# salvatore373/Humanoid-Navigation-using-MPC-LDCBF

Measured on AMD Instinct MI355X. Metric: MPC-step QP solves/sec (batch) at N=8, 10 obstacles, higher is better.
Workload: dtype f64

## Files before the change

### humanoid-navigation-using-mpc-ldcbf_amd/csrc/lipmpc_comm.hpp

```cpp
#pragma once
#include "lipmpc_types.hpp"

namespace lipmpc_dev {

#ifndef STREAM_UNROLL
#define STREAM_UNROLL 5
#endif
template <int I, int E, class F> __device__ __forceinline__ void static_for(F&& f) {
  if constexpr (I < E) {
    f(std::integral_constant<int, I>{});
    static_for<I + 1, E>(f);
  }
}
template <int I, int E, class F> __device__ __forceinline__ void static_rfor(F&& f) {
  if constexpr (I > E) {
    f(std::integral_constant<int, I - 1>{});
    static_rfor<I - 1, E>(f);
  }
}

__device__ __forceinline__ int fresh(int x) {
  asm volatile("" : "+v"(x));
  return x;
}
template <int CTRL, int BANK = 0xf, class T> __device__ __forceinline__ T dpp0(T x) {
  return __builtin_amdgcn_mov_dpp(x, CTRL, 0xf, BANK, true);
}
template <int M, class T> __device__ __forceinline__ T row_xor(T x) {
  if constexpr (M == 1) return dpp0<0xB1>(x);
  else if constexpr (M == 2) return dpp0<0x4E>(x);
  else if constexpr (M == 4) {
    T r = __builtin_amdgcn_mov_dpp(x, 0x104, 0xf, 0x5, false);
    return __builtin_amdgcn_update_dpp(r, x, 0x114, 0xf, 0xA, false);
  } else return dpp0<0x128>(x);
}
template <class T> __device__ __forceinline__ void rowpair(T v, T& even_rep, T& odd_rep) {
  if constexpr (sizeof(T) == 8) {
    const unsigned long long u = __builtin_bit_cast(unsigned long long, v);
    const unsigned lo = (unsigned)u, hi = (unsigned)(u >> 32);
    const auto a = __builtin_amdgcn_permlane16_swap(lo, lo, false, false);
    const auto b = __builtin_amdgcn_permlane16_swap(hi, hi, false, false);
    even_rep = __builtin_bit_cast(T, ((unsigned long long)b[0] << 32) | a[0]);
    odd_rep = __builtin_bit_cast(T, ((unsigned long long)b[1] << 32) | a[1]);
  } else {
    const unsigned u = __builtin_bit_cast(unsigned, v);
    const auto a = __builtin_amdgcn_permlane16_swap(u, u, false, false);
    const unsigned a0 = a[0], a1 = a[1];
    even_rep = __builtin_bit_cast(T, a0);
    odd_rep = __builtin_bit_cast(T, a1);
  }
}
template <class T> __device__ __forceinline__ T rowswap(T v) {
  T e, o;
  rowpair(v, e, o);
  const T r = (fresh(threadIdx.x) & 16) ? e : o;
  return r;
}
template <int G, int M, class T> __device__ __forceinline__ T gxor(T x) {
  if constexpr (M < 16) return row_xor<M>(x);
  else return rowswap(x);
}
template <int G, int J> __device__ __forceinline__ double gbcast(double x) {
  const double t = __builtin_amdgcn_mov_dpp(x, 0x150 + (J & 15), 0xf, 0xf, false);
  if constexpr (G == 16) return t;
  else {
    double e, o;
    rowpair(t, e, o);
    return (J < 16) ? e : o;
  }
}
template <int G, int D> __device__ __forceinline__ double gup(double x, int lane_) {
  const int lane = (G == 16) ? lane_ : fresh(lane_);
  if constexpr (G == 16) return dpp0<0x110 + D>(x);
  else if constexpr (D == 16) { const double w = rowswap(x); return (lane & 16) ? w : 0.0; }
  else {
    const double t = dpp0<0x120 + D>(x);
    const double w = rowswap(t);
    return ((lane & 15) >= D) ? t : ((lane & 16) ? w : 0.0);
  }
}
template <int G, int D> __device__ __forceinline__ double gdown(double x, int lane_) {
  const int lane = (G == 16) ? lane_ : fresh(lane_);
  if constexpr (G == 16) return dpp0<0x100 + D>(x);
  else if constexpr (D == 16) { const double w = rowswap(x); return (lane & 16) ? 0.0 : w; }
  else {
    const double t = dpp0<0x120 + (16 - D)>(x);
    const double w = rowswap(t);
    return ((lane & 15) + D < 16) ? t : ((lane & 16) ? 0.0 : w);
  }
}

template <int G> __device__ __forceinline__ double gsum(double x) {
  x += gxor<G, 1>(x); x += gxor<G, 2>(x); x += gxor<G, 4>(x); x += gxor<G, 8>(x);
  if constexpr (G == 32) x += gxor<G, 16>(x);
  return x;
}
__device__ __forceinline__ double vmax(double a, double b) {
  double r;
  asm("v_max_f64 %0, %1, %2" : "=v"(r) : "v"(a), "v"(b));
  return r;
}
__device__ __forceinline__ double vmin(double a, double b) {
  double r;
  asm("v_min_f64 %0, %1, %2" : "=v"(r) : "v"(a), "v"(b));
  return r;
}
__device__ __forceinline__ double vmax_abs(double m, double x) {
  double r;
  asm("v_max_f64 %0, %1, |%2|" : "=v"(r) : "v"(m), "v"(x));
  return r;
}
__device__ __forceinline__ double vmax0_abs(double x) {
  double r;
  asm("v_max_f64 %0, 0, |%1|" : "=v"(r) : "v"(x));
  return r;
}
__device__ __forceinline__ double vmax0(double x) {
  double r;
  asm("v_max_f64 %0, 0, %1" : "=v"(r) : "v"(x));
  return r;
}
template <int G> __device__ __forceinline__ double gmin(double x) {
  x = vmin(x, gxor<G, 1>(x)); x = vmin(x, gxor<G, 2>(x));
  x = vmin(x, dpp0<0x124>(x));
  x = vmin(x, gxor<G, 8>(x));
  if constexpr (G == 32) x = vmin(x, gxor<G, 16>(x));
  return x;
}
template <int G> __device__ __forceinline__ int gmin_int(int x) {
  x = min(x, gxor<G, 1>(x)); x = min(x, gxor<G, 2>(x)); x = min(x, dpp0<0x124>(x)); x = min(x, gxor<G, 8>(x));
  if constexpr (G == 32) x = min(x, gxor<G, 16>(x));
  return x;
}
template <int G> __device__ __forceinline__ double gmax(double x) {
  x = vmax(x, gxor<G, 1>(x)); x = vmax(x, gxor<G, 2>(x));
  x = vmax(x, dpp0<0x124>(x));
  x = vmax(x, gxor<G, 8>(x));
  if constexpr (G == 32) x = vmax(x, gxor<G, 16>(x));
  return x;
}
template <int G, int M> __device__ __forceinline__ void gargmin_step(double& v, int& i) {
  const double ov = gxor<G, M>(v);
  const int oi = gxor<G, M>(i);
  const bool take = (ov < v) || (ov == v && oi < i);
  v = take ? ov : v;
  i = take ? oi : i;
}
template <int G> __device__ __forceinline__ void gargmin(double& v, int& i) {
  gargmin_step<G, 1>(v, i); gargmin_step<G, 2>(v, i); gargmin_step<G, 4>(v, i); gargmin_step<G, 8>(v, i);
  if constexpr (G == 32) gargmin_step<G, 16>(v, i);
}
template <int G> __device__ __forceinline__ double prefix_excl2(double v, int lane) {
  double s = v;
  s += gup<G, 2>(s, lane); s += gup<G, 4>(s, lane); s += gup<G, 8>(s, lane);
  if constexpr (G == 32) s += gup<G, 16>(s, lane);
  return s - v;
}
template <int G> __device__ __forceinline__ double suffix_excl2(double v, int lane) {
  double s = v;
  s += gdown<G, 2>(s, lane); s += gdown<G, 4>(s, lane); s += gdown<G, 8>(s, lane);
  if constexpr (G == 32) s += gdown<G, 16>(s, lane);
  return s - v;
}
__device__ __forceinline__ double fast_rsqrt(double x) {
  double y = __builtin_amdgcn_rsq(x);
  y = y * fma(-0.5 * x * y, y, 1.5);
  y = y * fma(-0.5 * x * y, y, 1.5);
  return y;
}
__device__ __forceinline__ double fast_rcp(double x) {
  double y = __builtin_amdgcn_rcp(x);
  return fma(fma(-x, y, 1.0), y, y);
}
__device__ __forceinline__ double chain_rcp(double x) { return fast_rcp(x); }

template <int J> __device__ __forceinline__ double fmac_bcast_self(double acc, double mult) {
  asm("s_nop 1\n\tv_fmac_f64_dpp %0, %0, %1 row_newbcast:%2 row_mask:0xf bank_mask:0xf" : "+v"(acc) : "v"(mult), "n"(J));
  return acc;
}
__device__ __forceinline__ void dpp_fence() { asm volatile("s_nop 4"); }
#include "lipmpc_fused_steps.inc"

__device__ __forceinline__ double zero_unless(bool c, double x) {
  const unsigned long long u = __builtin_bit_cast(unsigned long long, x);
  const unsigned hi = c ? (unsigned)(u >> 32) : 0u;
  return __builtin_bit_cast(double, ((unsigned long long)hi << 32) | (unsigned)u);
}
#ifdef LIPMPC_PHASE_TIMING
constexpr int PH_WORDS = 32;
__device__ __forceinline__ void ph_mark(unsigned long long* acc, int k, int G) {
  const unsigned long long now = wall_clock64();
  const unsigned long long live = __ballot(1);
  if ((int)threadIdx.x == __ffsll((long long)live) - 1) {
    const unsigned long long dt = now - acc[31];
    acc[k] += dt;
    if (__popcll(live) <= G) acc[12 + k] += dt;
    acc[31] = now;
  }
  __builtin_amdgcn_fence(__ATOMIC_ACQ_REL, "workgroup");
  __builtin_amdgcn_wave_barrier();
}
#define PH_DECL __shared__ unsigned long long ph_acc_[PH_WORDS];                                                   \
  if (threadIdx.x == 0) { for (int k_ = 0; k_ < PH_WORDS; ++k_) ph_acc_[k_] = 0ull; ph_acc_[31] = in.t_start_wall; }     \
  __builtin_amdgcn_fence(__ATOMIC_ACQ_REL, "workgroup"); __builtin_amdgcn_wave_barrier();
#define PH(k) ph_mark(ph_acc_, k, G);
#else
#define PH_DECL
#define PH(k)
#endif
constexpr int WAVE = 64;
__device__ __forceinline__ void wave_sync() {
  __builtin_amdgcn_fence(__ATOMIC_ACQ_REL, "workgroup");
  __builtin_amdgcn_wave_barrier();
}
__device__ __forceinline__ double lds_read_here(const double* p) {
  return *(const volatile __attribute__((address_space(3))) double*)p;
}
struct RowFlags {
  unsigned m = 0u;
  __device__ __forceinline__ bool operator[](int i) const { return (m >> i) & 1u; }
  __device__ __forceinline__ void set(int i, bool v) { m = v ? (m | (1u << i)) : (m & ~(1u << i)); }
};

}
```

### humanoid-navigation-using-mpc-ldcbf_amd/csrc/lipmpc_solve.hpp

```cpp
#pragma once
#include "lipmpc_front.hpp"

namespace lipmpc_dev {

template <int G, int NOBS_L, int NVAR = G, bool LEAN = false, bool RECORD = false>
__device__ __forceinline__ StepOut step_solve(
    const KArgs& P, const StepIn& in, const FrontOut<G>& F, const double (*obs)[4], const int* perm,
    double* __restrict__ U, double* __restrict__ X, double* __restrict__ obj_out, int32_t* __restrict__ status_out,
    int32_t* __restrict__ iters_out, unsigned long long* __restrict__ active_out,
    unsigned long long* __restrict__ working_out,
    double* __restrict__ diag, WarmIO* __restrict__ warm, int32_t* __restrict__ cost_out) {
  static_assert(NVAR == G || (G == 16 && NVAR == 8), "variable slots: all lanes, or the first 8 of a 16-lane group");
  constexpr int NMAX = NVAR / 2;
  constexpr int LMAX = G / 2;
  constexpr int NV = NVAR;
  constexpr int GPW = 64 / G;
  constexpr bool STREAM = NOBS_L > 7;
  constexpr int NOBS_R = STREAM ? 0 : NOBS_L;
  constexpr int NOBS_S = STREAM ? NOBS_L : 0;
  constexpr int NR = R_CBF + NOBS_R;
  constexpr int MAXOBS = 2 * NOBS_L;
  constexpr int MAXWORDS = 16;
  constexpr bool FUSED = (G == 16);
  constexpr bool FUSED32 = (G == 32);
  constexpr bool FUSED32_SOLVE = FUSED32 && NOBS_L <= 2 && !LEAN;

  __shared__ double lds_P[GPW][LMAX][2][2];
  __shared__ unsigned long long lds_act[GPW][MAXWORDS];
  __shared__ double lds_mu[GPW][2];
  __shared__ double lds_sz[GPW][NOBS_S > 0 ? NOBS_S : 1][G][2];

  PH_DECL
  const int tid = threadIdx.x;
  const int lane = tid & (G - 1);
  const int grp = tid / G;
  const bool valid = in.valid;
  const long pb = in.pb;
  const int N = P.N;
  const int a = lane >> 1;
  const int c = lane & 1;
  const bool var_on = a < N;
  const double sgn_a = (a & 1) ? -1.0 : 1.0;
  const double kap = P.kappa;

  const double p0x = in.p0x, v0x = in.v0x, p0y = in.p0y, v0y = in.v0y, th0 = in.th0;
  const double gx = in.gx, gy = in.gy, foot0 = in.foot0, delta = in.delta;
  const double p0c = c ? p0y : p0x, v0c = c ? v0y : v0x, gc = c ? gy : gx;

  const double th_r = F.th_r, th_v = F.th_v, om_a = F.om_a, theta1 = F.theta1, omega0 = F.omega0;
  const double s_own = F.s_own, c_own = F.c_own;
  (void)th_r; (void)th_v;
  const double s_oth = gxor<G, 1>(s_own), c_oth = gxor<G, 1>(c_own);
  const double sr = c ? s_oth : s_own, cr = c ? c_oth : c_own, sv = c ? s_own : s_oth, cv = c ? c_own : c_oth;
  const double foot_r = (a & 1) ? -foot0 : foot0;
  const double foot_v = -foot_r;
  const double on = var_on ? 1.0 : 0.0;
  const double ro = on * cr, rq = on * (c ? -sr : sr);
  const double wo = on * (c ? cv * foot_v : cv), wq = on * (c ? -sv : sv);
  const double cm = (c == 0) ? on : 0.0;
  const double kap_l = on * kap;

  const int front_flag = F.front_flag;
  const double n_ball = F.n_ball, s_ball = F.s_ball;
  const bool ball = (lane == 1) && (n_ball > 0.0);
  const double ball_w = ball ? n_ball - 1.0 : 0.0;

  double oo[NOBS_R > 0 ? NOBS_R : 1], oq[NOBS_R > 0 ? NOBS_R : 1], ob[NOBS_R > 0 ? NOBS_R : 1];
  RowFlags pres;
#pragma unroll
  for (int t = 0; t < NOBS_R; ++t) {
    const int j = 2 * t + c;
    const bool there = var_on && ((double)(a + 1) >= obs[j][3]);
    const double ex = obs[j][0], ey = obs[j][1];
    oo[t] = there ? (c ? ey : ex) : 0.0; oq[t] = there ? (c ? ex : ey) : 0.0;
    ob[t] = there ? obs[j][2] : -1.0;
    pres.set(R_CBF + t, there);
  }
  unsigned pbits = 0u;
#pragma unroll
  for (int t = 0; t < NOBS_S; ++t)
    if (var_on && (double)(a + 1) >= obs[2 * t + c][3]) pbits |= 1u << t;
  auto s_obs = [&](int t, double& ex, double& ey, double& b) {
    const double* o = obs[2 * t + c];
    ex = o[0]; ey = o[1]; b = o[2];
  };
  auto s_pm = [&](int t) -> double { return ((pbits >> t) & 1u) ? 1.0 : 0.0; };
  pres.set(R_RU, var_on); pres.set(R_RL, var_on); pres.set(R_VU, var_on); pres.set(R_VL, var_on);
  pres.set(R_M, (var_on && (c == 0)) || ball);

  const double hi_r = P.l_max[c], lo_r = P.l_min[c];
  const double hi_v = c ? in.vmax_y : in.vmax_x, lo_v = P.v_min[c];
  const double hi_m = in.vmax_x - in.alpha_over_pi * fabs(om_a);
  const double p0q = c ? p0x : p0y, v0q = c ? v0x : v0y;
  const double r_c = (c ? foot_r * P.ell : 0.0) - ((a == 0) ? (ro * p0c + rq * p0q) : 0.0);
  const double w_c = wo * (-sgn_a * (v0c + kap * p0c)) + wq * (-sgn_a * (v0q + kap * p0q));

  int n_rows_l = __popc(pbits);
#pragma unroll
  for (int i = 0; i < NR; ++i) n_rows_l += pres[i] ? 1 : 0;
  const double m_rows = gsum<G>((double)n_rows_l) + fmax(n_ball - 1.0, 0.0);
  const double inv_m = 1.0 / fmax(m_rows, 1.0);

#include "lipmpc_solve_ops.inc"
#include "lipmpc_solve_ipm.inc"
#include "lipmpc_solve_finish.inc"
#include "lipmpc_solve_outputs.inc"
  StepOut r;
  r.status = status; r.iters = iters; r.theta1 = theta1; r.omega0 = omega0; r.obj = objv;
  r.ux = gbcast<G, 0>(u); r.uy = gbcast<G, 1>(u);
  return r;
}


}
```

### humanoid-navigation-using-mpc-ldcbf_amd/csrc/lipmpc_solve_finish.inc

```
  if (ball) { pres.set(R_M, false); s[R_M] = 1.0; z[R_M] = 0.0; }
  if (warm_on) {
    wave_sync();
    warm->lds[lane] = q;
#pragma unroll
    for (int i = 0; i < NR && i < WARM_ROWS; ++i) {
      if constexpr (RECORD) warm->lds[(1 + i) * G + lane] = pres[i] ? z[i] : 0.0;
      else warm->lds[(1 + i) * G + lane] = z[i];
    }
    wave_sync();
  }
  const CanonicalRows ci_of{a, c, N, P, perm};
  auto ci_s = [&](int t) -> int { return ci_of.ldcbf(t); };

  double marg_l = INFINITY;
  const bool want_diag = diag != nullptr;
  RowFlags act;
  unsigned abits = 0u;
#pragma unroll
  for (int i = 0; i < NR; ++i) {
    if (want_diag && pres[i]) marg_l = fmin(marg_l, fabs(log(z[i] / (FIN_IDENT * s[i]))));
    act.set(i, pres[i] && (z[i] > FIN_IDENT * s[i]));
  }
  if constexpr (STREAM) {
#pragma unroll STREAM_UNROLL
    for (int t = 0; t < NOBS_S; ++t) {
      if ((pbits >> t) & 1u) {
        const double st = lds_sz[grp][t][lane][0], zt = lds_sz[grp][t][lane][1];
        if (want_diag) marg_l = fmin(marg_l, fabs(log(zt / (FIN_IDENT * st))));
        if (zt > FIN_IDENT * st) abits |= 1u << t;
      }
    }
  }
  const unsigned fbits = abits;
  const double margin = gmin<G>(marg_l);
  double diag_rounds = 0.0, diag_eres = 0.0, diag_cert = 0.0;

  const bool ipm_ok = (status == LIPMPC_STATUS_SOLVED) && (m_rows > 0.0);
  if (!(P.flags & LIPMPC_FLAG_INTERIOR)) {
    bool fin_done = !ipm_ok;
    bool certified = false;
    double rho = FIN_RHO;
    double xf = q;
    double qf = q;
    double y[NR];
#pragma unroll
    for (int i = 0; i < NR; ++i) y[i] = act[i] ? z[i] : 0.0;
    if constexpr (STREAM) {
#pragma unroll STREAM_UNROLL
      for (int t = 0; t < NOBS_S; ++t)
        if (!((abits >> t) & 1u)) lds_sz[grp][t][lane][1] = 0.0;
    }
    auto s_slack = [&](int t, double fx, double fy) -> double {
#pragma clang fp contract(off)
      double ex, ey, bb;
      s_obs(t, ex, ey, bb);
      return ex * fx + ey * fy - bb;
    };
    auto s_ratio = [&](int t, double fx, double fy, double ddx, double ddy) -> double {
#pragma clang fp contract(off)
      double ex, ey, bb;
      s_obs(t, ex, ey, bb);
      const double sl = ex * fx + ey * fy - bb, gd = -(ex * ddx + ey * ddy);
      const bool cand = gd > FIN_GD_MIN;
      return cand ? fmax(sl + gd, 0.0) * fast_rcp(gd) : INFINITY;
    };
    for (int rnd = 0; rnd < P.fin_rounds; ++rnd) {
      if (__all(fin_done)) break;
      double d[NR];
#pragma unroll
      for (int i = 0; i < NR; ++i) d[i] = act[i] ? rho : 0.0;
      double cxs = 0.0, cxys = 0.0, cys = 0.0;
      if constexpr (STREAM) {
#pragma unroll STREAM_UNROLL
        for (int t = 0; t < NOBS_S; ++t) {
          if ((abits >> t) & 1u) {
            double ex, ey, bb;
            s_obs(t, ex, ey, bb);
            cxs = fma(rho * ex, ex, cxs); cxys = fma(rho * ex, ey, cxys); cys = fma(rho * ey, ey, cys);
          }
        }
      }
      PH(9)
      K_rows(d, cxs, cxys, cys);
      const bool fok = factor();
      PH(7)
      qf = xf;
      double eres = INFINITY, rd_g = 0.0, r_g = 0.0;
      for (int in = 0; in <= FIN_INNER; ++in) {
        slack_values(qf);
        const double fx = cx_, fy = cy_;
        double wr[NR], rmax_l = 0.0;
#pragma unroll
        for (int i = 0; i < NR; ++i) {
          const double r = act[i] ? -slk[i] : 0.0;
          wr[i] = -d[i] * slk[i];
          rmax_l = i == 0 ? vmax0_abs(r) : vmax_abs(rmax_l, r);
        }
        double ayx = 0.0, ayy = 0.0, awx = 0.0, awy = 0.0;
        if constexpr (STREAM) {
#pragma unroll STREAM_UNROLL
          for (int t = 0; t < NOBS_S; ++t) {
            if ((abits >> t) & 1u) {
              double ex, ey, bb;
              s_obs(t, ex, ey, bb);
              const double r = -(ex * fx + ey * fy - bb);
              const double yt = lds_sz[grp][t][lane][1];
              rmax_l = fmax(rmax_l, fabs(r));
              ayx = fma(ex, yt, ayx); ayy = fma(ey, yt, ayy);
              awx = fma(ex, rho * r, awx); awy = fma(ey, rho * r, awy);
            }
          }
        }
        const double gty = GT_rows(y, ayx, ayy);
        const double rd = var_on ? (2.0 * (qf - gc) + gty) : 0.0;
        const double eprev = eres;
        rd_g = gmax<G>(fabs(rd));
        r_g = gmax<G>(rmax_l);
        eres = vmax(rd_g, r_g);
        const bool stop = (eres <= FIN_INNER_TOL) || (in == FIN_INNER) || (eres <= FIN_EPS && eres > FIN_STALL * eprev);
        if (__all(stop || fin_done)) break;
        const double dq = solve(-rd - GT_rows(wr, awx, awy));
        double dl[NR];
        rows_dir(dq, dl);
        if (!stop && !fin_done) {
          qf += dq;
#pragma unroll
          for (int i = 0; i < NR; ++i) y[i] = fma(d[i], dl[i] - slk[i], y[i]);
          if constexpr (STREAM) {
            const double ddx = cx_, ddy = cy_;
#pragma unroll STREAM_UNROLL
            for (int t = 0; t < NOBS_S; ++t) {
              if ((abits >> t) & 1u) {
                double ex, ey, bb;
                s_obs(t, ex, ey, bb);
                const double slk_t = ex * fx + ey * fy - bb, dl_t = -(ex * ddx + ey * ddy);
                lds_sz[grp][t][lane][1] += rho * (dl_t - slk_t);
              }
            }
          }
        }
      }
      PH(8)
      const double fx = cx_, fy = cy_;
      const double dd = qf - xf;
      double gd[NR], rr[NR];
      rows_dir(dd, gd);
      const double ddx = cx_, ddy = cy_;
      double rbest = INFINITY;
#pragma unroll
      for (int i = 0; i < NR; ++i) {
        const bool cand = pres[i] & !act[i] & (gd[i] > FIN_GD_MIN);
        rr[i] = cand ? fmax(slk[i] + gd[i], 0.0) * fast_rcp(gd[i]) : INFINITY;
        rbest = fmin(rbest, rr[i]);
      }
      double ymin = INFINITY, ymax = 0.0, smin = INFINITY;
#pragma unroll
      for (int i = 0; i < NR; ++i) {
        const bool ta = act[i], ti = pres[i] & !ta;
        const double ylo = ta ? y[i] : INFINITY, yhi = ta ? y[i] : 0.0, slo = ti ? slk[i] : INFINITY;
        ymin = i == 0 ? fmin(ymin, ylo) : vmin(ymin, ylo);
        ymax = i == 0 ? vmax0(yhi) : vmax(ymax, yhi);
        smin = i == 0 ? fmin(smin, slo) : vmin(smin, slo);
      }
      if constexpr (STREAM) {
#pragma unroll STREAM_UNROLL
        for (int t = 0; t < NOBS_S; ++t) {
          if ((pbits >> t) & 1u) {
            if ((abits >> t) & 1u) { const double yt = lds_sz[grp][t][lane][1]; ymin = fmin(ymin, yt); ymax = fmax(ymax, yt); }
            else { smin = fmin(smin, s_slack(t, fx, fy)); rbest = fmin(rbest, s_ratio(t, fx, fy, ddx, ddy)); }
          }
        }
      }
      rbest = gmin<G>(rbest);
      ymin = gmin<G>(ymin);
      int bi = 0x7fffffff;
      const bool blocked = !fin_done & (rbest < 1.0);
      const bool dropping = !fin_done & !blocked & (ymin < -FIN_EPS);
      if (__any(blocked)) {
#pragma unroll
        for (int i = 0; i < NR; ++i) {
          const int ci = ci_of(i);
          bi = ((rr[i] == rbest) & (ci < bi)) ? ci : bi;
        }
        if constexpr (STREAM) {
#pragma unroll STREAM_UNROLL
          for (int t = 0; t < NOBS_S; ++t) {
            if (((pbits >> t) & 1u) && !((abits >> t) & 1u)) {
              const int ci = ci_s(t);
              if (s_ratio(t, fx, fy, ddx, ddy) == rbest && ci < bi) bi = ci;
            }
          }
        }
        bi = gmin_int<G>(bi);
      }
      if (__any(blocked | dropping)) {
#pragma unroll
        for (int i = 0; i < NR; ++i) {
          const bool hd = dropping & act[i] & (y[i] < -FIN_EPS), ha = blocked & pres[i] & !act[i] & (ci_of(i) == bi);
          y[i] = hd ? 0.0 : y[i];
          act.m = (act.m & ~((unsigned)hd << i)) | ((unsigned)ha << i);
        }
        if constexpr (STREAM) {
#pragma unroll STREAM_UNROLL
          for (int t = 0; t < NOBS_S; ++t) {
            const bool on_t = (pbits >> t) & 1u, act_t = (abits >> t) & 1u;
            if (dropping && act_t && lds_sz[grp][t][lane][1] < -FIN_EPS) { abits &= ~(1u << t); lds_sz[grp][t][lane][1] = 0.0; }
            if (blocked && on_t && !act_t && ci_s(t) == bi) abits |= 1u << t;
          }
        }
      }
      if (!fin_done) {
        if (blocked) {
          xf = fma(rbest, dd, xf);
        } else {
          xf = qf;
          const bool polish = !dropping & (eres > FIN_POLISH_TOL) & (rho == FIN_RHO) & (rnd + 1 < P.fin_rounds);
          rho = polish ? FIN_RHO_POLISH : rho;
          if (!dropping && !polish) {
            ymax = gmax<G>(ymax);
            smin = gmin<G>(smin);
            const double qabs = gmax<G>(fabs(qf));
            fin_done = true;
            certified = fok && (r_g <= FIN_EPS) && (rd_g <= FIN_EPS + FIN_DUAL_REL * ymax) && (smin >= -FIN_EPS) && (qabs < 1e300);
            diag_cert = vmin(ymin, smin);
          }
        }
        diag_rounds = rnd + 1;
        diag_eres = eres;
      }
    }
    if (ipm_ok) {
      if (certified) {
        q = xf;
      } else {
        status = LIPMPC_STATUS_UNCERTIFIED;
#pragma unroll
        for (int i = 0; i < NR; ++i) act.set(i, pres[i] && (z[i] > FIN_IDENT * s[i]));
        abits = fbits;
      }
    }
  }

  PH(9)
```

### humanoid-navigation-using-mpc-ldcbf_amd/csrc/lipmpc_solve_ipm.inc

```
  const bool warm_on = warm != nullptr && warm->lds != nullptr;
  const bool warm_in = warm_on && warm->have;
  const bool last_stage = a >= N - 1;
  const int wsrc = last_stage ? lane : lane + 2;
  double q = var_on ? p0c : 0.0;
  if (warm_in) {
    const double qo = warm->lds[lane], qn = warm->lds[wsrc], qb = warm->lds[lane >= 2 ? lane - 2 : lane];
    q = var_on ? (last_stage ? qo + (qo - qb) : qn) : 0.0;
  }
  double s[NR], z[NR], slk[NR];
  double hl[NOBS_R > 0 ? NOBS_R : 1];
  double cx_ = 0.0, cy_ = 0.0;
  auto slack_values = [&](double x) {
    double r_lin, w_lin;
    rows_lin(x, r_lin, w_lin, hl, cx_, cy_);
    const double r = r_lin + r_c, w = w_lin + w_c;
    slk[R_RU] = hi_r - r; slk[R_RL] = r - lo_r;
    slk[R_VU] = hi_v - w; slk[R_VL] = w - lo_v;
    slk[R_M] = hi_m - w;
#pragma unroll
    for (int t = 0; t < NOBS_R; ++t) slk[R_CBF + t] = hl[t] - ob[t];
  };
  auto rows_dir = [&](double dx, double (&dl)[NR]) {
    double r_lin, w_lin;
    rows_lin(dx, r_lin, w_lin, hl, cx_, cy_);
    dl[R_RU] = r_lin; dl[R_RL] = -r_lin; dl[R_VU] = w_lin; dl[R_VL] = -w_lin; dl[R_M] = cm * w_lin;
#pragma unroll
    for (int t = 0; t < NOBS_R; ++t) dl[R_CBF + t] = -hl[t];
  };
  auto GT_rows = [&](const double (&w)[NR], double axs, double ays) -> double {
    double wc[NOBS_R > 0 ? NOBS_R : 1];
#pragma unroll
    for (int t = 0; t < NOBS_R; ++t) wc[t] = w[R_CBF + t];
    return GT_apply(w[R_RU] - w[R_RL], fma(cm, w[R_M], w[R_VU] - w[R_VL]), wc, axs, ays);
  };
  auto K_rows = [&](const double (&d)[NR], double cxs, double cxys, double cys) {
    double dc[NOBS_R > 0 ? NOBS_R : 1];
#pragma unroll
    for (int t = 0; t < NOBS_R; ++t) dc[t] = d[R_CBF + t];
    form_K(d[R_RU] + d[R_RL], fma(cm, d[R_M], d[R_VU] + d[R_VL]), dc, cxs, cxys, cys);
  };

  slack_values(q);
  slk[R_M] = ball ? s_ball : slk[R_M];
#pragma unroll
  for (int i = 0; i < NR; ++i) {
    slk[i] = pres[i] ? slk[i] : 1.0;
    s[i] = pres[i] ? fmax(slk[i], IPM_S_FLOOR) : 1.0;
    z[i] = pres[i] ? IPM_Z0 : 1e-300;
    if (warm_in && i < WARM_ROWS) z[i] = pres[i] ? fmin(fmax(warm->lds[(1 + i) * G + wsrc], WARM_Z_MIN), WARM_Z_MAX) : 1e-300;
  }
  if constexpr (STREAM) {
#pragma unroll STREAM_UNROLL
    for (int t = 0; t < NOBS_S; ++t) {
      double ex, ey, b;
      s_obs(t, ex, ey, b);
      const bool on = (pbits >> t) & 1u;
      lds_sz[grp][t][lane][0] = on ? fmax(ex * cx_ + ey * cy_ - b, IPM_S_FLOOR) : 1.0;
      lds_sz[grp][t][lane][1] = on ? IPM_Z0 : 0.0;
    }
  }
  struct SRow { double s, z, rp, is, d, ex, ey, pm; };
  auto s_row = [&](int t, double px, double py) -> SRow {
    SRow r;
    double b;
    s_obs(t, r.ex, r.ey, b);
    r.pm = s_pm(t);
    r.s = lds_sz[grp][t][lane][0]; r.z = lds_sz[grp][t][lane][1];
    r.rp = (r.s - (r.ex * px + r.ey * py - b)) * r.pm;
    r.is = fast_rcp(r.s);
    r.d = r.z * r.is;
    return r;
  };

  int status = LIPMPC_STATUS_MAX_ITER;
  int iters = 0;
  bool done = false;
  if (front_flag & 2) { status = LIPMPC_STATUS_DEGENERATE; done = true; }
  else if (front_flag & 1) { status = LIPMPC_STATUS_INFEASIBLE; done = true; }
  if (in.sensor_overflow) { status = LIPMPC_STATUS_SENSOR_OVERFLOW; done = true; }
  if (front_flag & 8) { status = LIPMPC_STATUS_MAX_ITER; done = true; }
  if (m_rows == 0.0 && !done) { status = LIPMPC_STATUS_SOLVED; done = true; q = var_on ? gc : 0.0; }

  double pm[NR];
#pragma unroll
  for (int i = 0; i < NR; ++i) pm[i] = pres[i] ? 2.0 : 1.0;

  double rp[NR];
#pragma unroll
  for (int i = 0; i < NR; ++i) rp[i] = s[i] - slk[i];
  if (lane == 0) { lds_mu[grp][0] = INFINITY; lds_mu[grp][1] = 0.0; }
  PH(10)
  for (int it = 0; it <= P.max_iter; ++it) {
    if (__all(done)) break;
    if (!done) {
      const double mu_prev = lds_read_here(&lds_mu[grp][0]);
      double w[NR], d[NR];
      double mu_l = 0.0, rpmax_l = 0.0, zmax_l = 0.0;
#pragma unroll
      for (int i = 0; i < NR; ++i) {
        mu_l = fma(s[i], z[i], mu_l);
        rpmax_l = i == 0 ? vmax0_abs(rp[i]) : vmax_abs(rpmax_l, rp[i]);
        zmax_l = i == 0 ? vmax0(z[i]) : vmax(zmax_l, z[i]);
      }
      mu_l = fma(ball_w * s[R_M], z[R_M], mu_l);
      double qx = 0.0, qy = 0.0, cxs = 0.0, cxys = 0.0, cys = 0.0, axs = 0.0, ays = 0.0;
      if constexpr (STREAM) {
        const double qp = gxor<G, 1>(q);
        qx = c ? qp : q; qy = c ? q : qp;
#pragma unroll STREAM_UNROLL
        for (int t = 0; t < NOBS_S; ++t) {
          const SRow r = s_row(t, qx, qy);
          mu_l = fma(r.s, r.z, mu_l);
          rpmax_l = fmax(rpmax_l, fabs(r.rp));
          zmax_l = fmax(zmax_l, r.z);
          cxs = fma(r.d * r.ex, r.ex, cxs); cxys = fma(r.d * r.ex, r.ey, cxys); cys = fma(r.d * r.ey, r.ey, cys);
          const double wt = fma(r.d, r.rp - r.s, r.z);
          axs = fma(r.ex, wt, axs); ays = fma(r.ey, wt, ays);
        }
      }
      const double musum = gsum<G>(mu_l);
      const double mu = musum * inv_m;
      double mu_prev_in = mu_prev;
      asm volatile("" : "+v"(mu_prev_in) : "v"(mu));
      {
        const double ramp = fmin(1.0, fmax(0.0, (mu * __builtin_amdgcn_rcp(mu_prev_in) - IPM_SLOW_RATIO) * (1.0 / (1.0 - IPM_SLOW_RATIO))));
        if (lane == 0) { lds_mu[grp][0] = mu; lds_mu[grp][1] = (it >= IPM_SLOW_FROM) ? IPM_SLOW_SIGMA * ramp : 0.0; }
      }
      const double zq_l = fmax(zmax_l * (1.0 / IPM_Z_DIVERGE), fabs(q) * 1e-300);
      const double rpmax = gmax<G>(!(zq_l < 1.0) ? INFINITY : rpmax_l);
      const bool bad = !(rpmax < INFINITY);
      if (rpmax <= P.tol && mu <= P.tol) { status = LIPMPC_STATUS_SOLVED; done = true; iters = it; }
      else if (it == P.max_iter) { done = true; iters = it; }
      else if (bad) { status = LIPMPC_STATUS_INFEASIBLE; done = true; iters = it; }
      PH(0)
      if (!done) {
        double is_[NR];
#pragma unroll
        for (int i = 0; i < NR; ++i) {
          const double y0 = __builtin_amdgcn_rcp(s[i]);
          is_[i] = y0 * fma(-s[i], y0, pm[i]);
          d[i] = z[i] * is_[i];
        }
        K_rows(d, cxs, cxys, cys);
        PH(1)
        const bool fok = factor();
        PH(2)
        if (!fok) {
          status = (rpmax <= IPM_STALL_TOL && mu <= IPM_STALL_TOL) ? LIPMPC_STATUS_SOLVED : LIPMPC_STATUS_INFEASIBLE;
          done = true; iters = it;
        }
        const double m2qg = var_on ? -2.0 * (q - gc) : 0.0;
#pragma unroll
        for (int i = 0; i < NR; ++i) w[i] = fma(d[i], rp[i] - s[i], z[i]);
        const double dqa = solve(m2qg - GT_rows(w, axs, ays));
        const double sigma_floor = lds_read_here(&lds_mu[grp][1]);
        PH(3)
        double dl[NR], c2[NR];
        rows_dir(dqa, dl);
        const double ax_ = cx_, ay_ = cy_;
        double r_l = 1.0;
        double s2_l = 0.0;
#pragma unroll
        for (int i = 0; i < NR; ++i) {
          const double dsa = -rp[i] - dl[i];
          const double t = dsa * is_[i];
          const double dza = -fma(d[i], dsa, z[i]);
          r_l = fmax(r_l, fmax(-t, 1.0 + t));
          c2[i] = dsa * dza;
          s2_l += c2[i];
        }
        s2_l = fma(ball_w, c2[R_M], s2_l);
        if constexpr (STREAM) {
#pragma unroll STREAM_UNROLL
          for (int t = 0; t < NOBS_S; ++t) {
            const SRow r = s_row(t, qx, qy);
            const double dsa_t = (-r.rp + (r.ex * ax_ + r.ey * ay_)) * r.pm;
            const double dza_t = -r.d * (r.s + dsa_t);
            r_l = fmax(r_l, fmax(-dsa_t * r.is, -dza_t * __builtin_amdgcn_rcp(fmax(r.z, 1e-300))));
            s2_l = fma(dsa_t, dza_t, s2_l);
          }
        }
        const double a_aff = chain_rcp(gmax<G>(r_l));
        const double mu_aff = fma(a_aff * a_aff, gsum<G>(s2_l), (1.0 - a_aff) * musum) * inv_m;
        const double ratio = mu_aff * chain_rcp(mu);
        double sigma = ratio * ratio * ratio;
        sigma = vmax(sigma, sigma_floor);
        const double sigma_mu = sigma * mu;
        PH(4)
        double rc[NR];
#pragma unroll
        for (int i = 0; i < NR; ++i) {
          rc[i] = fma(s[i], z[i], c2[i]) - sigma_mu;
          w[i] = fma(fma(z[i], rp[i], -rc[i]), is_[i], z[i]);
        }
        axs = 0.0; ays = 0.0;
        if constexpr (STREAM) {
#pragma unroll STREAM_UNROLL
          for (int t = 0; t < NOBS_S; ++t) {
            const SRow r = s_row(t, qx, qy);
            const double dsa_t = (-r.rp + (r.ex * ax_ + r.ey * ay_)) * r.pm;
            const double dza_t = -r.d * (r.s + dsa_t);
            const double rc_t = (fma(r.s, r.z, dsa_t * dza_t) - sigma_mu) * r.pm;
            const double wt = fma(fma(r.z, r.rp, -rc_t), r.is, r.z);
            axs = fma(r.ex, wt, axs); ays = fma(r.ey, wt, ays);
          }
        }
        const double dq = solve(m2qg - GT_rows(w, axs, ays));
        PH(5)
        rows_dir(dq, dl);
        const double bx_ = cx_, by_ = cy_;
        r_l = IPM_STEP_FRAC;
        double ds[NR], dz[NR];
#pragma unroll
        for (int i = 0; i < NR; ++i) {
          ds[i] = -rp[i] - dl[i];
          dz[i] = -fma(z[i], ds[i], rc[i]) * is_[i];
          r_l = fmax(r_l, fmax(-ds[i] * is_[i], -dz[i] * __builtin_amdgcn_rcp(z[i])));
        }
        auto s_step = [&](const SRow& r, double& ds_t, double& dz_t) {
          const double dsa_t = (-r.rp + (r.ex * ax_ + r.ey * ay_)) * r.pm;
          const double dza_t = -r.d * (r.s + dsa_t);
          const double rc_t = (fma(r.s, r.z, dsa_t * dza_t) - sigma_mu) * r.pm;
          ds_t = (-r.rp + (r.ex * bx_ + r.ey * by_)) * r.pm;
          dz_t = -fma(r.z, ds_t, rc_t) * r.is;
        };
        if constexpr (STREAM) {
#pragma unroll STREAM_UNROLL
          for (int t = 0; t < NOBS_S; ++t) {
            const SRow r = s_row(t, qx, qy);
            double ds_t, dz_t;
            s_step(r, ds_t, dz_t);
            r_l = fmax(r_l, fmax(-ds_t * r.is, -dz_t * __builtin_amdgcn_rcp(fmax(r.z, 1e-300))));
          }
        }
        const double alpha = IPM_STEP_FRAC * chain_rcp(gmax<G>(r_l));
        if (!done) {
          if constexpr (STREAM) {
#pragma unroll STREAM_UNROLL
            for (int t = 0; t < NOBS_S; ++t) {
              const SRow r = s_row(t, qx, qy);
              double ds_t, dz_t;
              s_step(r, ds_t, dz_t);
              lds_sz[grp][t][lane][0] = fma(alpha, ds_t, r.s);
              lds_sz[grp][t][lane][1] = fma(alpha, dz_t, r.z);
            }
          }
          q = fma(alpha, dq, q);
          const double oma = 1.0 - alpha;
#pragma unroll
          for (int i = 0; i < NR; ++i) {
            s[i] = fma(alpha, ds[i], s[i]); z[i] = fma(alpha, dz[i], z[i]); rp[i] *= oma;
          }
        }
        PH(6)
      }
    }
  }
```

Baseline: 44.46 million.

## Park loop-invariant slack constants in AGPRs and simplify finish-phase selects

```diff
diff --git a/humanoid-navigation-using-mpc-ldcbf_amd/csrc/lipmpc_comm.hpp b/humanoid-navigation-using-mpc-ldcbf_amd/csrc/lipmpc_comm.hpp
--- a/humanoid-navigation-using-mpc-ldcbf_amd/csrc/lipmpc_comm.hpp
+++ b/humanoid-navigation-using-mpc-ldcbf_amd/csrc/lipmpc_comm.hpp
@@ -186,6 +186,16 @@
   const unsigned hi = c ? (unsigned)(u >> 32) : 0u;
   return __builtin_bit_cast(double, ((unsigned long long)hi << 32) | (unsigned)u);
 }
+__device__ __forceinline__ double nan_unless(bool c, double x) {
+  const unsigned long long u = __builtin_bit_cast(unsigned long long, x);
+  const unsigned hi = c ? (unsigned)(u >> 32) : 0xffffffffu;
+  return __builtin_bit_cast(double, ((unsigned long long)hi << 32) | (unsigned)u);
+}
+__device__ __forceinline__ double vmin_inf(double x) {
+  double r;
+  asm("v_min_f64 %0, %1, %2" : "=v"(r) : "s"((double)INFINITY), "v"(x));
+  return r;
+}
 #ifdef LIPMPC_PHASE_TIMING
 constexpr int PH_WORDS = 32;
 __device__ __forceinline__ void ph_mark(unsigned long long* acc, int k, int G) {
@@ -216,6 +226,7 @@
 __device__ __forceinline__ double lds_read_here(const double* p) {
   return *(const volatile __attribute__((address_space(3))) double*)p;
 }
+__device__ __forceinline__ void park(double& x) { asm volatile("" : "+a"(x)); }
 struct RowFlags {
   unsigned m = 0u;
   __device__ __forceinline__ bool operator[](int i) const { return (m >> i) & 1u; }
diff --git a/humanoid-navigation-using-mpc-ldcbf_amd/csrc/lipmpc_solve.hpp b/humanoid-navigation-using-mpc-ldcbf_amd/csrc/lipmpc_solve.hpp
--- a/humanoid-navigation-using-mpc-ldcbf_amd/csrc/lipmpc_solve.hpp
+++ b/humanoid-navigation-using-mpc-ldcbf_amd/csrc/lipmpc_solve.hpp
@@ -88,12 +88,12 @@
   pres.set(R_RU, var_on); pres.set(R_RL, var_on); pres.set(R_VU, var_on); pres.set(R_VL, var_on);
   pres.set(R_M, (var_on && (c == 0)) || ball);
 
-  const double hi_r = P.l_max[c], lo_r = P.l_min[c];
-  const double hi_v = c ? in.vmax_y : in.vmax_x, lo_v = P.v_min[c];
-  const double hi_m = in.vmax_x - in.alpha_over_pi * fabs(om_a);
+  double hi_r = P.l_max[c], lo_r = P.l_min[c];
+  double hi_v = c ? in.vmax_y : in.vmax_x, lo_v = P.v_min[c];
+  double hi_m = in.vmax_x - in.alpha_over_pi * fabs(om_a);
   const double p0q = c ? p0x : p0y, v0q = c ? v0x : v0y;
-  const double r_c = (c ? foot_r * P.ell : 0.0) - ((a == 0) ? (ro * p0c + rq * p0q) : 0.0);
-  const double w_c = wo * (-sgn_a * (v0c + kap * p0c)) + wq * (-sgn_a * (v0q + kap * p0q));
+  double r_c = (c ? foot_r * P.ell : 0.0) - ((a == 0) ? (ro * p0c + rq * p0q) : 0.0);
+  double w_c = wo * (-sgn_a * (v0c + kap * p0c)) + wq * (-sgn_a * (v0q + kap * p0q));
 
   int n_rows_l = __popc(pbits);
 #pragma unroll
diff --git a/humanoid-navigation-using-mpc-ldcbf_amd/csrc/lipmpc_solve_finish.inc b/humanoid-navigation-using-mpc-ldcbf_amd/csrc/lipmpc_solve_finish.inc
--- a/humanoid-navigation-using-mpc-ldcbf_amd/csrc/lipmpc_solve_finish.inc
+++ b/humanoid-navigation-using-mpc-ldcbf_amd/csrc/lipmpc_solve_finish.inc
@@ -92,7 +92,7 @@
         double wr[NR], rmax_l = 0.0;
 #pragma unroll
         for (int i = 0; i < NR; ++i) {
-          const double r = act[i] ? -slk[i] : 0.0;
+          const double r = nan_unless(act[i], slk[i]);
           wr[i] = -d[i] * slk[i];
           rmax_l = i == 0 ? vmax0_abs(r) : vmax_abs(rmax_l, r);
         }
@@ -150,17 +150,17 @@
 #pragma unroll
       for (int i = 0; i < NR; ++i) {
         const bool cand = pres[i] & !act[i] & (gd[i] > FIN_GD_MIN);
-        rr[i] = cand ? fmax(slk[i] + gd[i], 0.0) * fast_rcp(gd[i]) : INFINITY;
-        rbest = fmin(rbest, rr[i]);
+        rr[i] = nan_unless(cand, fmax(slk[i] + gd[i], 0.0) * fast_rcp(gd[i]));
+        rbest = i == 0 ? vmin_inf(rr[i]) : vmin(rbest, rr[i]);
       }
       double ymin = INFINITY, ymax = 0.0, smin = INFINITY;
 #pragma unroll
       for (int i = 0; i < NR; ++i) {
         const bool ta = act[i], ti = pres[i] & !ta;
-        const double ylo = ta ? y[i] : INFINITY, yhi = ta ? y[i] : 0.0, slo = ti ? slk[i] : INFINITY;
-        ymin = i == 0 ? fmin(ymin, ylo) : vmin(ymin, ylo);
-        ymax = i == 0 ? vmax0(yhi) : vmax(ymax, yhi);
-        smin = i == 0 ? fmin(smin, slo) : vmin(smin, slo);
+        const double ya = nan_unless(ta, y[i]), so = nan_unless(ti, slk[i]);
+        ymin = i == 0 ? vmin_inf(ya) : vmin(ymin, ya);
+        ymax = i == 0 ? vmax0(ya) : vmax(ymax, ya);
+        smin = i == 0 ? vmin_inf(so) : vmin(smin, so);
       }
       if constexpr (STREAM) {
 #pragma unroll STREAM_UNROLL
@@ -174,32 +174,38 @@
       rbest = gmin<G>(rbest);
       ymin = gmin<G>(ymin);
       int bi = 0x7fffffff;
+      unsigned bw = 0u;
       const bool blocked = !fin_done & (rbest < 1.0);
       const bool dropping = !fin_done & !blocked & (ymin < -FIN_EPS);
       if (__any(blocked)) {
 #pragma unroll
         for (int i = 0; i < NR; ++i) {
-          const int ci = ci_of(i);
-          bi = ((rr[i] == rbest) & (ci < bi)) ? ci : bi;
+          const int key = (ci_of(i) << 4) | i;
+          bi = ((rr[i] == rbest) & (key < bi)) ? key : bi;
         }
         if constexpr (STREAM) {
 #pragma unroll STREAM_UNROLL
           for (int t = 0; t < NOBS_S; ++t) {
             if (((pbits >> t) & 1u) && !((abits >> t) & 1u)) {
-              const int ci = ci_s(t);
-              if (s_ratio(t, fx, fy, ddx, ddy) == rbest && ci < bi) bi = ci;
+              const int key = (ci_s(t) << 4) | 15;
+              if (s_ratio(t, fx, fy, ddx, ddy) == rbest && key < bi) bi = key;
             }
           }
         }
+        const int key_l = bi;
         bi = gmin_int<G>(bi);
+        bw = (key_l == bi) ? (1u << (bi & 15)) : 0u;
+        if constexpr (STREAM) { bw &= (1u << NR) - 1u; bi >>= 4; }
       }
       if (__any(blocked | dropping)) {
+        unsigned dm = 0u;
 #pragma unroll
         for (int i = 0; i < NR; ++i) {
-          const bool hd = dropping & act[i] & (y[i] < -FIN_EPS), ha = blocked & pres[i] & !act[i] & (ci_of(i) == bi);
+          const bool hd = dropping & act[i] & (y[i] < -FIN_EPS);
           y[i] = hd ? 0.0 : y[i];
-          act.m = (act.m & ~((unsigned)hd << i)) | ((unsigned)ha << i);
-        }
+          dm |= (unsigned)hd << i;
+        }
+        act.m = (act.m & ~dm) | (blocked ? bw : 0u);
         if constexpr (STREAM) {
 #pragma unroll STREAM_UNROLL
           for (int t = 0; t < NOBS_S; ++t) {
diff --git a/humanoid-navigation-using-mpc-ldcbf_amd/csrc/lipmpc_solve_ipm.inc b/humanoid-navigation-using-mpc-ldcbf_amd/csrc/lipmpc_solve_ipm.inc
--- a/humanoid-navigation-using-mpc-ldcbf_amd/csrc/lipmpc_solve_ipm.inc
+++ b/humanoid-navigation-using-mpc-ldcbf_amd/csrc/lipmpc_solve_ipm.inc
@@ -89,6 +89,12 @@
 #pragma unroll
   for (int i = 0; i < NR; ++i) rp[i] = s[i] - slk[i];
   if (lane == 0) { lds_mu[grp][0] = INFINITY; lds_mu[grp][1] = 0.0; }
+  auto park_slack_constants = [&]() {
+    park(hi_r); park(lo_r); park(hi_v); park(lo_v); park(hi_m); park(r_c); park(w_c);
+#pragma unroll
+    for (int t = 0; t < NOBS_R; ++t) park(ob[t]);
+  };
+  park_slack_constants();
   PH(10)
   for (int it = 0; it <= P.max_iter; ++it) {
     if (__all(done)) break;
@@ -256,3 +262,4 @@
       }
     }
   }
+  park_slack_constants();
```

New measurement: 44.70 million (median of 2 runs). Within noise of the previous version (+0.5%).
